# RobertKajnak/AMT-SAGA

Measured on AMD Instinct MI355X. Metric: audio windows/sec (44.1 kHz, 2048-pt STFT) through full detect->subtract loop, higher is better.
Workload: dtype f32 (conv: split-fp16 x2 operands, f32 accumulate; 4x16 layers on the large images in the FFT domain); 1 GPU; C3: 1024 polyphonic piano windows, STFT(2048) + pitch+velocity+timing(start,end) heads + 1 subtraction iteration; windows_per_gpu=1024, n_fft=2048, hop=512, frames=516, iters=1, parallelism=windows sharded x1, event all-gather

## Files before the change

### amt-saga_amd/csrc/amt_conv_f16x3.h

```cpp
#pragma once

typedef _Float16 f16x8 __attribute__((ext_vector_type(8)));
typedef unsigned int u32x2 __attribute__((ext_vector_type(2)));
typedef float f32x4 __attribute__((ext_vector_type(4)));
#define HX_PSTRIDE 80
#define HXS_NIT 2
#define HX_TPITCH 36
#define HX_LSCALE 2048.0f
#define HX_MINNORM 6.103515625e-05f

__host__ __device__ __forceinline__ unsigned short amt_f16_bits(_Float16 h) {
    unsigned short b;
    __builtin_memcpy(&b, &h, 2);
    return b;
}
template <bool FLUSH>
__host__ __device__ __forceinline__ void amt_split_f16(float xs, unsigned short &hb, unsigned short &lb) {
    _Float16 h = (_Float16)xs;
    if (FLUSH && !(__builtin_fabsf(xs) >= HX_MINNORM)) h = (_Float16)0.0f;
    const float r = (xs - (float)h) * HX_LSCALE;
    _Float16 l = (_Float16)r;
    if (FLUSH && !(__builtin_fabsf(r) >= HX_MINNORM)) l = (_Float16)0.0f;
    hb = amt_f16_bits(h);
    lb = amt_f16_bits(l);
// ... 203 lines not shown
            asm volatile("s_waitcnt vmcnt(0)" ::: "memory");
#pragma unroll
            for (int i = 0; i < WPT; ++i) reinterpret_cast<u32x4 *>(wbuf)[tid + i * NT] = wp[i];
            if (NGT > 1) issue(1);
        }
        __syncthreads();
        if (tsp && tid == 0 && ch == 0) tsp[1] = wall_clock64();
        union U { uint4 u; f16x8 v; };
#pragma unroll 1
        for (int g = 0; g < NG; ++g) {
            const int gg = ch * NG + g;
            const uint4 *wb = wbuf + (gg & 1) * GV4 + lane;
            U a[2];
            U b[2][2];
            auto loadA = [&](int tp, int ms) {
                const int tap = g * GT + 2 * tp;
                const int dy = tap / KW, dx = tap - dy * KW;
                const char *ap;
                if constexpr (MASKED) {
                    const int rr = (int)(lrc[ms] & 255u) + dy - PAD_T;
                    const int cc = (int)((lrc[ms] >> 8) & 255u) + dx + tsel - PAD_L;
                    const bool inb = (unsigned)rr < (unsigned)p.H && (unsigned)cc < (unsigned)p.W;
                    ap = in_lds + (inb ? abase[ms] + ((dy - PAD_T) * RP + (dx + tsel - PAD_L)) * HX_PSTRIDE : zero_off);
                } else {
                    ap = in_lds + abase[ms] + (dy * RP + dx) * HX_PSTRIDE;
                }
                a[0].u = *reinterpret_cast<const uint4 *>(ap);
                a[1].u = *reinterpret_cast<const uint4 *>(ap + 32);
            };
            auto mfma6 = [&](int ms) {
#pragma unroll
                for (int ns = 0; ns < 2; ++ns) {
                    lo[ms][ns] = __builtin_amdgcn_mfma_f32_16x16x32_f16(a[1].v, b[ns][0].v, lo[ms][ns], 0, 0, 0);
                    hi[ms][ns] = __builtin_amdgcn_mfma_f32_16x16x32_f16(a[0].v, b[ns][0].v, hi[ms][ns], 0, 0, 0);
                    lo[ms][ns] = __builtin_amdgcn_mfma_f32_16x16x32_f16(a[0].v, b[ns][1].v, lo[ms][ns], 0, 0, 0);
                }
            };
            if constexpr (!MASKED) if (g == NG - 1 && ch + 1 < NCHUNK) stage_issue(ch + 1);
#pragma unroll
            for (int tp = 0; tp < GT / 2; ++tp) {
#pragma unroll
                for (int ns = 0; ns < 2; ++ns)
#pragma unroll
                    for (int pl = 0; pl < 2; ++pl) b[ns][pl].u = wb[((tp * 2 + pl) * 2 + ns) * 64];
#pragma unroll
                for (int ms = 0; ms < MS; ++ms) {
                    loadA(tp, ms);
                    mfma6(ms);
                }
            }
            __builtin_amdgcn_sched_barrier(0);
            if (gg + 1 < NGT) {
                asm volatile("s_waitcnt vmcnt(0)" ::: "memory");
                u32x4 *dst = reinterpret_cast<u32x4 *>(wbuf + ((gg + 1) & 1) * GV4);
#pragma unroll
                for (int i = 0; i < WPT; ++i) dst[tid + i * NT] = wp[i];
                if (gg + 2 < NGT) issue(gg + 2);
            }
            if (g + 1 < NG) __syncthreads();
        }
    }
    if (tsp && tid == 0) tsp[2] = wall_clock64();
    if (tid < PCAP) {
        const int wl = min(max(pos_win[tid] - win0, 0), HX_MAXWIN - 1);
        const int sa = (int)(__float_as_uint(win_is[wl]) >> 23) - 127;
        const int sw = TRAIN ? *hs.sw_dev : hs.sw;
        pos_os[tid] = __uint_as_float((unsigned)(127 - (sa + sw)) << 23);
    }
    __syncthreads();
    float *tb = reinterpret_cast<float *>(in_lds) + wid * (16 * MS * HX_TPITCH);
    const int c4 = (lane & 7) * 4;
    const float4 s2v = *reinterpret_cast<const float4 *>(bnp + 64 + c4), t2v = *reinterpret_cast<const float4 *>(bnp + 96 + c4);
    float osc[MS][4];
#pragma unroll
    for (int ms = 0; ms < MS; ++ms)
#pragma unroll
        for (int e = 0; e < 4; ++e) osc[ms][e] = pos_os[wid * (16 * MS) + ms * 16 + 4 * (lane >> 4) + e];
#pragma unroll
    for (int ns = 0; ns < 2; ++ns) {
        const float s1 = bnp[ns * 16 + (lane & 15)], t1 = bnp[32 + ns * 16 + (lane & 15)];
#pragma unroll
        for (int ms = 0; ms < MS; ++ms)
#pragma unroll
            for (int e = 0; e < 4; ++e) {
                const int row = ms * 16 + 4 * (lane >> 4) + e;
                const float z = (hi[ms][ns][e] + lo[ms][ns][e] * (1.0f / HX_LSCALE)) * osc[ms][e];
                tb[row * HX_TPITCH + ns * 16 + (lane & 15)] = TRAIN ? z + t1 : sigmoidf_(z * s1 + t1);
            }
    }
    constexpr int NR = 2 * MS;
    int spq[NR], gwq[NR];
    float4 scv[NR];
#pragma unroll
    for (int i = 0; i < NR; ++i) {
        const int q = wid * (16 * MS) + (lane >> 3) + 8 * i;
        spq[i] = pos_sp[q];
        gwq[i] = pos_win[q];
    }
    const bool has_sc = p.sc || p.sc1;
    if (p.sc) {
#pragma unroll
        for (int i = 0; i < NR; ++i) {
            const float *scp = p.sc + (size_t)gwq[i] * p.sc_win_stride + (size_t)max(spq[i], 0) * p.cout_total + cout_off + c4;
            scv[i] = spq[i] >= 0 ? *reinterpret_cast<const float4 *>(scp) : make_float4(0.f, 0.f, 0.f, 0.f);
        }
    } else if (p.sc1) {
        const float4 w4 = *reinterpret_cast<const float4 *>(p.sc1_w + cout_off + c4);
        const float4 s4 = *reinterpret_cast<const float4 *>(p.sc1_s + cout_off + c4);
        const float4 t4 = *reinterpret_cast<const float4 *>(p.sc1_t + cout_off + c4);
#pragma unroll
        for (int i = 0; i < NR; ++i) {
            const float x = spq[i] >= 0 ? p.sc1[(size_t)gwq[i] * p.sc1_win_stride + spq[i]] : 0.f;
            scv[i] = make_float4(fmaf(x, w4.x, 0.f) * s4.x + t4.x, fmaf(x, w4.y, 0.f) * s4.y + t4.y,
                                 fmaf(x, w4.z, 0.f) * s4.z + t4.z, fmaf(x, w4.w, 0.f) * s4.w + t4.w);
        }
    }
    float rmax[NR];
#pragma unroll
    for (int i = 0; i < NR; ++i) {
        float4 v = *reinterpret_cast<const float4 *>(tb + ((lane >> 3) + 8 * i) * HX_TPITCH + c4);
        rmax[i] = 0.f;
        if (spq[i] < 0) continue;
        if (has_sc) {
            v.x = (v.x + scv[i].x) * s2v.x + t2v.x;
            v.y = (v.y + scv[i].y) * s2v.y + t2v.y;
            v.z = (v.z + scv[i].z) * s2v.z + t2v.z;
            v.w = (v.w + scv[i].w) * s2v.w + t2v.w;
        }
        rmax[i] = fmaxf(fmaxf(fabsf(v.x), fabsf(v.y)), fmaxf(fabsf(v.z), fabsf(v.w)));
        *reinterpret_cast<float4 *>(p.out + (size_t)gwq[i] * p.out_win_stride + (size_t)spq[i] * p.cout_total + cout_off + c4) = v;
    }
    if (hs.amax_out) {
        if (p.NWIN == 1) {
            float m = 0.f;
#pragma unroll
            for (int i = 0; i < NR; ++i) m = fmaxf(m, rmax[i]);
            m = wave_max(m);
            if (lane == 0) atomicMax(win_max, __float_as_int(m));
        } else {
#pragma unroll
            for (int i = 0; i < NR; ++i) {
                float m = rmax[i];
                m = fmaxf(m, __shfl_xor(m, 1, 64));
                m = fmaxf(m, __shfl_xor(m, 2, 64));
                m = fmaxf(m, __shfl_xor(m, 4, 64));
                if ((lane & 7) == 0 && spq[i] >= 0) atomicMax(win_max + (gwq[i] - win0), __float_as_int(m));
            }
        }
        __syncthreads();
        if (tid < p.NWIN && win0 + tid < p.B) atomicMax(reinterpret_cast<int *>(hs.amax_out) + win0 + tid, win_max[tid]);
    }
    if (tsp && tid == 0) tsp[3] = wall_clock64();
}
```

### amt-saga_amd/csrc/amt_rdcnn.hip

```cpp
#include "amt_common.h"
#include "amt_fftconv.h"
#include "amt_convh.h"
#include "amt_rdcnn_topology.h"
#include <vector>
#include <algorithm>
#include <cmath>
#include <cstdlib>

#include "amt_conv_f32.h"
#include "amt_conv_bf16x6.h"
#include "amt_conv_f16x3.h"
#include "amt_rdcnn_small.h"

#define RD_BN_EPS 1e-3f

struct ConvPlan {
    int TH = 0, TW = 0, NWIN = 1;
    size_t lds = 0;
    int nslice = 1, cw = 0;
    bool masked = false;
    double eff = 0;
    void *w = nullptr;
};
struct ConvOp {
    int cin, cout, H, W, kh, kw;
    float *s1 = nullptr, *t1 = nullptr, *s2 = nullptr, *t2 = nullptr;
    bool residual = false;
    int sc_proj = -1;
    int pool_after = 0;
    ConvPlan f32;
    int MT = 2;
    ConvPlan bf16;
    ConvPlan f16;
    int sw = 0;
    std::vector<float> k_host;
    FcLayer fc;
};
struct ProjOp {
    int cin, cout, H, W, ph, pw, HO, WO;
    float *w = nullptr, *s = nullptr, *t = nullptr;
};
struct Tower {
    int in_h, in_w, ph, pw;
    std::vector<ConvOp> convs;
    std::vector<ProjOp> projs;
    size_t max_act = 0;
    int out_h, out_w, out_c;
};
struct ProfPending { hipEvent_t e0, e1; int tower, layer, windows; };
struct ProfAcc { double ms = 0, windows = 0; long launches = 0; };
struct amt_rdcnn {
    mutable bool prof_on = false;
    mutable std::vector<ProfPending> prof_pending;
    mutable std::vector<hipEvent_t> prof_free;
    mutable std::vector<std::vector<ProfAcc>> prof_acc;
    amt_rdcnn_desc d;
    std::vector<Tower> towers;
    std::vector<void *> allocs;
    float *d1w = nullptr, *d1b = nullptr, *d2w = nullptr, *d2b = nullptr;
    int flat = 0;
    double flops = 0;
    mutable int mode = 0;
};

template <class T>
static int upload(amt_rdcnn *n, const void *h, size_t bytes, T **out) {
    void *d = nullptr;
    if (hipMalloc(&d, bytes) != hipSuccess) return AMT_E_NOMEM;
    n->allocs.push_back(d);
    if (hipMemcpy(d, h, bytes, hipMemcpyHostToDevice) != hipSuccess) return AMT_E_HIP;
    *out = static_cast<T *>(d);
    return AMT_OK;
}
static int upload_folded_bn(amt_rdcnn *n, const float *bn, int c, const float *bias, float **s_out, float **t_out) {
    const float *g = bn, *b = bn + c, *m = bn + 2 * c, *v = bn + 3 * c;
    std::vector<float> s(c), t(c);
    for (int i = 0; i < c; ++i) {
        const float sc = g[i] / sqrtf(v[i] + RD_BN_EPS);
        s[i] = sc;
        t[i] = b[i] + ((bias ? bias[i] : 0.f) - m[i]) * sc;
    }
    const int rc = upload(n, s.data(), c * sizeof(float), s_out);
    return rc != AMT_OK ? rc : upload(n, t.data(), c * sizeof(float), t_out);
}

template <class F>
static void for_each_tile(int H, int W, int pcap, int max_win, F consider) {
    if (H * W <= pcap)
        for (int nw = std::min(pcap / (H * W), max_win); nw >= 1; --nw) consider(H, W, nw);
    for (int TH = 1; TH <= H && TH <= pcap; ++TH) {
        int TW = pcap / TH;
        if (TW > W) TW = W;
        if (TW >= 1) consider(TH, TW, 1);
        const int nct = (W + TW - 1) / TW;
        const int TW2 = (W + nct - 1) / nct;
        if (TW2 >= 1 && TW2 <= TW) consider(TH, TW2, 1);
    }
}

static void choose_tile(ConvOp &c) {
    ConvPlan &p = c.f32;
    double best = -1;
    for (int MT = 2; MT >= 1; --MT) {
        const int pcap = 128 * MT;
        for_each_tile(c.H, c.W, pcap, pcap, [&](int TH, int TW, int NWIN) {
            const size_t posin = (size_t)NWIN * (TH + c.kh - 1) * (TW + c.kw - 1);
            const size_t lds = posin * RD_CSTRIDE * 4 + 2 * (size_t)RD_CC * p.cw * 4 + (size_t)pcap * 8;
            if (lds > 150 * 1024) return;
            const double tiles = (double)((c.H + TH - 1) / TH) * ((c.W + TW - 1) / TW) / NWIN;
            double eff = (double)c.H * c.W / (tiles * pcap);
            if (lds > 78 * 1024) eff *= 0.93;
            if (eff > best + 1e-9) { best = eff; p.TH = TH; p.TW = TW; p.NWIN = NWIN; c.MT = MT; p.lds = lds; p.eff = eff; }
        });
    }
}

template <class F>
static void choose_tile_split(const ConvOp &c, ConvPlan &p, int max_win, F lds_of) {
    double best = -1;
    const int pcap = 256;
    p.masked = false; p.TH = 0;
    if (c.H * c.W <= 64) {
        const int nw = std::min(pcap / (c.H * c.W), max_win);
        const size_t lds = lds_of((size_t)nw * c.H * c.W + 1);
        if (lds <= 79 * 1024) {
            p.masked = true; p.TH = c.H; p.TW = c.W; p.NWIN = nw; p.lds = lds;
            p.eff = (double)nw * c.H * c.W / pcap;
            return;
        }
    }
    for_each_tile(c.H, c.W, pcap, max_win, [&](int TH, int TW, int NWIN) {
        const size_t lds = lds_of((size_t)NWIN * (TH + c.kh - 1) * bx_row_pitch(TW, TW + c.kw - 1));
        if (lds > 79 * 1024) return;
        const double tiles = (double)((c.H + TH - 1) / TH) * ((c.W + TW - 1) / TW) / NWIN;
        const double eff = (double)c.H * c.W / (tiles * pcap);
        if (eff > best + 1e-9) { best = eff; p.TH = TH; p.TW = TW; p.NWIN = NWIN; p.lds = lds; p.eff = eff; }
    });
}
static void choose_tile16(ConvOp &c) {
    const int NT = c.bf16.cw / 32, ntaps = c.kh * c.kw;
    const int tps = (NT == 1 && ntaps % 2 == 0) ? 2 : 1;
    const size_t slab = (size_t)tps * 3 * NT * 64 * 16;
    choose_tile_split(c, c.bf16, 256, [&](size_t npos) { return npos * BX_PSTRIDE + 3 * slab + (size_t)256 * 8; });
}

static unsigned apply_plan(ConvParams &p, const ConvPlan &pl) {
    p.TH = pl.TH; p.TW = pl.TW; p.NWIN = pl.NWIN;
    p.tiles_h = (p.H + p.TH - 1) / p.TH; p.tiles_w = (p.W + p.TW - 1) / p.TW;
    const int groups = (p.B + p.NWIN - 1) / p.NWIN;
    return (unsigned)((size_t)groups * p.tiles_h * p.tiles_w);
}

template <int KH, int KW, int CIN, int COUT, bool MASKED>
static int launch_conv16_t(const ConvOp &c, ConvParams p, hipStream_t st) {
    auto kern = conv_bf16x6_kernel<KH, KW, CIN, COUT, MASKED>;
    static bool attr_set = false;
    if (!attr_set) {
        AMT_HIP_CHECK(hipFuncSetAttribute(reinterpret_cast<const void *>(kern),
                                          hipFuncAttributeMaxDynamicSharedMemorySize, (int)(80 * 1024)));
        attr_set = true;
    }
    const unsigned grid = apply_plan(p, c.bf16);
    kern<<<dim3(grid, c.bf16.nslice), 512, c.bf16.lds, st>>>(p, static_cast<const uint4 *>(c.bf16.w));
    AMT_LAUNCH_CHECK();
    return AMT_OK;
}
template <int KH, int KW>
static int launch_conv16_k(const ConvOp &c, const ConvParams &p, hipStream_t st) {
#define BX_CASE(CI, CO)                                                              \
    if (c.cin == CI && c.bf16.cw == CO)                                              \
        return c.bf16.masked ? launch_conv16_t<KH, KW, CI, CO, true>(c, p, st)          \
                          : launch_conv16_t<KH, KW, CI, CO, false>(c, p, st);
    BX_CASE(32, 32) BX_CASE(32, 64) BX_CASE(64, 64) BX_CASE(128, 64)
#undef BX_CASE
    return AMT_E_UNSUPPORTED;
}
static bool conv_channels_supported(int cin, int cout) {
    return (cin == 32 && cout == 32) || (cin == 32 && cout == 64) || (cin == 64 && cout == 64) ||
           (cin == 64 && cout == 128) || (cin == 128 && cout == 128);
}
static int launch_conv16(const ConvOp &c, const ConvParams &p, hipStream_t st) {
    if (c.kh == 4 && c.kw == 16) return launch_conv16_k<4, 16>(c, p, st);
    if (c.kh == 4 && c.kw == 2) return launch_conv16_k<4, 2>(c, p, st);
    if (c.kh == 2 && c.kw == 2) return launch_conv16_k<2, 2>(c, p, st);
    return AMT_E_UNSUPPORTED;
}


#define HX_SLAB_BYTES 4096
#define HX_XCHG_BYTES (8 * 32 * HX_TPITCH * 4)
static void choose_tile_h(ConvOp &c) {
    const int NTh = c.f16.cw / 32;
    const int nsteps = c.kh * c.kw / (NTh == 1 ? 2 : 1);
    const size_t wbytes = 2 * (size_t)std::min(4, nsteps) * HX_SLAB_BYTES;
    choose_tile_split(c, c.f16, HX_MAXWIN, [&](size_t npos) {
        return std::max(npos * HX_PSTRIDE, (size_t)HX_XCHG_BYTES) + wbytes + (size_t)256 * 12 + (size_t)HX_MAXWIN * 8 + 512;
    });
}

template <int KH, int KW, int CIN, bool MASKED>
static int launch_convs_t(const ConvOp &c, ConvParams p, const float *amax_in, float *amax_out, hipStream_t st) {
    auto kern = conv_f16x3s_kernel<KH, KW, CIN, MASKED>;
    static bool attr_set = false;
    if (!attr_set) {
        AMT_HIP_CHECK(hipFuncSetAttribute(reinterpret_cast<const void *>(kern),
                                          hipFuncAttributeMaxDynamicSharedMemorySize, (int)(80 * 1024)));
        attr_set = true;
    }
    const unsigned grid = apply_plan(p, c.f16);
    HxScale hs{amax_in, amax_out, c.sw, nullptr};
    static const bool want_ts = getenv("AMT_CONV_TS") != nullptr;
    static unsigned long long *ts_dev = nullptr;
    static size_t ts_cap = 0;
    const size_t nwg = (size_t)grid * c.f16.nslice;
    if (want_ts) {
        if (nwg > ts_cap) {
            if (ts_dev) (void)hipFree(ts_dev);
            AMT_HIP_CHECK(hipMalloc(&ts_dev, nwg * 4 * sizeof(unsigned long long)));
            ts_cap = nwg;
        }
        hs.ts = ts_dev;
    }
    kern<<<dim3(grid, c.f16.nslice), 512, c.f16.lds, st>>>(p, static_cast<const uint4 *>(c.f16.w), hs);
    AMT_LAUNCH_CHECK();
    if (want_ts) {
        AMT_HIP_CHECK(hipStreamSynchronize(st));
        std::vector<unsigned long long> h(nwg * 4);
        AMT_HIP_CHECK(hipMemcpy(h.data(), ts_dev, h.size() * sizeof(unsigned long long), hipMemcpyDeviceToHost));
        double a = 0, b = 0, e = 0;
        unsigned long long t0 = ~0ull, t1 = 0;
        for (size_t i = 0; i < nwg; ++i) {
            a += (double)(h[4 * i + 1] - h[4 * i]); b += (double)(h[4 * i + 2] - h[4 * i + 1]);
            e += (double)(h[4 * i + 3] - h[4 * i + 2]);
            t0 = std::min(t0, h[4 * i]); t1 = std::max(t1, h[4 * i + 3]);
        }
        fprintf(stderr, "conv_ts k%dx%d cin%d %dx%d masked%d wgs %zu: start->first MFMA %.2f us, MFMA loop %.2f us, epilogue %.2f us; "
                        "kernel %.1f us = %.2f workgroup lives per slot of 512\n",
                KH, KW, CIN, p.H, p.W, (int)MASKED, nwg, a / nwg / 100.0, b / nwg / 100.0, e / nwg / 100.0,
                (double)(t1 - t0) / 100.0, (double)(t1 - t0) * 512.0 / ((a + b + e)));
    }
    return AMT_OK;
}
template <int KH, int KW>
static int launch_convh_k(const ConvOp &c, const ConvParams &p, const float *amax_in, float *amax_out, hipStream_t st) {
    if (!c.f16.w || c.f16.cw != 32) return AMT_E_UNSUPPORTED;
#define HXS_CASE(CI)                                                                       \
    if (c.cin == CI)                                                                       \
        return c.f16.masked ? launch_convs_t<KH, KW, CI, true>(c, p, amax_in, amax_out, st)               \
                            : launch_convs_t<KH, KW, CI, false>(c, p, amax_in, amax_out, st);
    HXS_CASE(32) HXS_CASE(64) HXS_CASE(128)
#undef HXS_CASE
    return AMT_E_UNSUPPORTED;
}
static int launch_convh(const ConvOp &c, const ConvParams &p, const float *amax_in, float *amax_out, hipStream_t st) {
    if (c.kh == 4 && c.kw == 16) return launch_convh_k<4, 16>(c, p, amax_in, amax_out, st);
    if (c.kh == 4 && c.kw == 2) return launch_convh_k<4, 2>(c, p, amax_in, amax_out, st);
    if (c.kh == 2 && c.kw == 2) return launch_convh_k<2, 2>(c, p, amax_in, amax_out, st);
    return AMT_E_UNSUPPORTED;
}

template <int KH, int KW, int CIN, int COUT, int MT>
static int launch_conv_t(const ConvOp &c, ConvParams p, hipStream_t st) {
    auto kern = conv_mfma_kernel<KH, KW, CIN, COUT, MT>;
    static size_t attr_set = 0;
    if (c.f32.lds > attr_set) {
        AMT_HIP_CHECK(hipFuncSetAttribute(reinterpret_cast<const void *>(kern),
                                          hipFuncAttributeMaxDynamicSharedMemorySize, (int)(152 * 1024)));
        attr_set = 152 * 1024;
    }
    const unsigned grid = apply_plan(p, c.f32);
    kern<<<dim3(grid, c.f32.nslice), 256, c.f32.lds, st>>>(p);
    AMT_LAUNCH_CHECK();
    return AMT_OK;
}

template <int KH, int KW>
static int launch_conv_k(const ConvOp &c, const ConvParams &p, hipStream_t st) {
#define RD_CASE(CI, CO)                                                         \
    if (c.cin == CI && c.f32.cw == CO)                                          \
        return c.MT == 2 ? launch_conv_t<KH, KW, CI, CO, 2>(c, p, st)           \
                         : launch_conv_t<KH, KW, CI, CO, 1>(c, p, st);
    RD_CASE(32, 32) RD_CASE(32, 64) RD_CASE(64, 64) RD_CASE(64, 128) RD_CASE(128, 128)
    RD_CASE(64, 32) RD_CASE(128, 32)
#undef RD_CASE
    return AMT_E_UNSUPPORTED;
}

static int launch_conv(const ConvOp &c, const ConvParams &p, hipStream_t st) {
    if (c.kh == 4 && c.kw == 16) return launch_conv_k<4, 16>(c, p, st);
    if (c.kh == 4 && c.kw == 2) return launch_conv_k<4, 2>(c, p, st);
    if (c.kh == 2 && c.kw == 2) return launch_conv_k<2, 2>(c, p, st);
    return AMT_E_UNSUPPORTED;
}

static void choose_tile1(int H, int W, int *TH_, int *TW_) {
    long best = -1;
    for (int TH = 1; TH <= H && TH <= C1M_PCAP; ++TH) {
        int TWmax = std::min(W, C1M_PCAP / TH);
        for (int TW = std::max(1, TWmax - 40); TW <= TWmax; ++TW) {
            const long tiles = (long)((H + TH - 1) / TH) * ((W + TW - 1) / TW);
            const long cost = tiles * ((TH * TW + 31) / 32);
            if (best < 0 || cost < best) { best = cost; *TH_ = TH; *TW_ = TW; }
        }
    }
}

static bool conv_supported(int kh, int kw) {
    return (kh == 4 && kw == 16) || (kh == 4 && kw == 2) || (kh == 2 && kw == 2);
}

static int launch_conv1_mfma(const ConvOp &c, const Conv1Params &cp, hipStream_t st) {
    int TH1 = 1, TW1 = 1;
    choose_tile1(cp.H, cp.W, &TH1, &TW1);
    const int th = (cp.H + TH1 - 1) / TH1, twn = (cp.W + TW1 - 1) / TW1;
    const size_t lds = (size_t)2 * C1M_PCAP * 4 + (size_t)4 * 32 * HX_TPITCH * 4 +
                       (size_t)(TH1 + c.kh - 1) * (TW1 + c.kw - 1) * 4;
    const unsigned grid = (unsigned)std::min<size_t>((size_t)cp.B * th * twn, 256 * 8);
    if (c.kh == 4 && c.kw == 16) conv1_mfma_kernel<4, 16><<<grid, 256, lds, st>>>(cp, TH1, TW1, th, twn);
    else if (c.kh == 4 && c.kw == 2) conv1_mfma_kernel<4, 2><<<grid, 256, lds, st>>>(cp, TH1, TW1, th, twn);
    else conv1_mfma_kernel<2, 2><<<grid, 256, lds, st>>>(cp, TH1, TW1, th, twn);
    AMT_LAUNCH_CHECK();
    return AMT_OK;
}
static int launch_conv1(const ConvOp &c, const Conv1Params &cp, hipStream_t st) {
    const int groups = 256 / c.cout;
    const size_t lds = ((size_t)c.kh * c.kw * c.cout +
                        (size_t)c.kh * (groups * C1_PPT + c.kw - 1)) * 4;
    const size_t tiles = (size_t)cp.B * cp.H * ((cp.W + groups * C1_PPT - 1) / (groups * C1_PPT));
    conv1_kernel<<<(unsigned)std::min<size_t>(tiles, 8192), 256, lds, st>>>(cp);
    AMT_LAUNCH_CHECK();
    return AMT_OK;
}

enum ConvImpl {
    IMPL_FIRST_MFMA,
    IMPL_FIRST_VALU,
    IMPL_FFT_ROW,
    IMPL_FFT_PACKED,
    IMPL_F16X3,
    IMPL_BF16X6,
    IMPL_F32
};
static ConvImpl conv_impl(const ConvOp &c, int mode) {
    if (c.cin == 1) return (c.cout == 32 && conv_supported(c.kh, c.kw)) ? IMPL_FIRST_MFMA : IMPL_FIRST_VALU;
    if (mode == 3 && c.fc.row) return IMPL_FFT_ROW;
    if (mode == 3 && c.fc.pk) return IMPL_FFT_PACKED;
    if (mode >= 2 && c.f16.w) return IMPL_F16X3;
    if (mode >= 1 && c.bf16.w) return IMPL_BF16X6;
    return IMPL_F32;
}
static bool impl_is_fft(ConvImpl impl) { return impl == IMPL_FFT_ROW || impl == IMPL_FFT_PACKED; }
static bool impl_forms_rank1_shortcut(ConvImpl impl, const ConvOp &c) {
    return impl == IMPL_FFT_ROW || (impl == IMPL_F16X3 && !c.f16.masked);
}
static bool impl_writes_amax(ConvImpl impl) {
    return impl == IMPL_FIRST_MFMA || impl_is_fft(impl) || impl == IMPL_F16X3;
}

static std::vector<float> pack_f32(const float *kern, int ntap, int C, int fo, int nslice) {
    const int nch = C / 32, cw = fo / nslice, NTW = cw / 32;
    std::vector<float> wa((size_t)ntap * C * fo);
    for (int sl = 0; sl < nslice; ++sl)
        for (int ch = 0; ch < nch; ++ch)
            for (int tap = 0; tap < ntap; ++tap)
                for (int cc = 0; cc < 32; ++cc)
                    for (int j = 0; j < 32; ++j)
                        for (int nt = 0; nt < NTW; ++nt)
                            wa[(((((size_t)sl * nch + ch) * ntap + tap) * 32 + cc) * 32 + j) * NTW + nt] =
                                kern[((size_t)tap * C + ch * 32 + cc) * fo + sl * cw + nt * 32 + j];
    return wa;
}
static std::vector<unsigned short> pack_bf16x6(const float *kern, int ntap, int C, int fo, int nslice16) {
    const int NT = fo / 32, cw16 = fo / nslice16, NT16 = cw16 / 32;
    const int tps = (NT16 == 1 && ntap % 2 == 0) ? 2 : 1;
    const int nslab = ntap / tps;
    const int nch16 = C / BX_CC;
    std::vector<unsigned short> w16((size_t)nch16 * ntap * 3 * NT * 2 * 32 * 8);
    for (int sl = 0; sl < nslice16; ++sl)
        for (int ch = 0; ch < nch16; ++ch)
            for (int sb = 0; sb < nslab; ++sb)
                for (int tt = 0; tt < tps; ++tt)
                    for (int nt = 0; nt < NT16; ++nt)
                        for (int h = 0; h < 2; ++h)
                            for (int col = 0; col < 32; ++col)
                                for (int jj = 0; jj < 8; ++jj) {
                                    const int tap = sb * tps + tt;
                                    const int cin_i = ch * BX_CC + 8 * h + jj;
                                    const float wv = kern[((size_t)tap * C + cin_i) * fo + sl * cw16 + nt * 32 + col];
                                    unsigned short hh[3];
                                    amt_split3(wv, hh[0], hh[1], hh[2]);
                                    for (int pl = 0; pl < 3; ++pl) {
                                        const size_t idx =
                                            ((((((((size_t)sl * nch16 + ch) * nslab + sb) * tps + tt) * 3 + pl) * NT16 + nt) * 2 + h) * 32 + col) * 8 + jj;
                                        w16[idx] = hh[pl];
                                    }
                                }
    return w16;
}
static std::vector<unsigned short> pack_f16x3(const float *kern, int ntap, int C, int fo, float wscale) {
    const int NT = fo / 32, nsliceh = fo / 32;
    const int nch16 = C / BX_CC;
    std::vector<unsigned short> ws((size_t)nch16 * ntap * 2 * NT * 2 * 32 * 8);
    const int ntp = ntap / 2;
    for (int sl = 0; sl < nsliceh; ++sl)
        for (int ch = 0; ch < nch16; ++ch)
            for (int tp = 0; tp < ntp; ++tp)
                for (int ns = 0; ns < 2; ++ns)
                    for (int ln = 0; ln < 64; ++ln)
                        for (int jj = 0; jj < 8; ++jj) {
                            const int col = ln & 15, kg = ln >> 4;
                            const int tap = 2 * tp + (kg & 1);
                            const int cin_i = ch * BX_CC + 8 * (kg >> 1) + jj;
                            const float wv = kern[((size_t)tap * C + cin_i) * fo + sl * 32 + ns * 16 + col];
                            unsigned short hh[2];
                            amt_split_f16<true>(wv * wscale, hh[0], hh[1]);
                            for (int pl = 0; pl < 2; ++pl) {
                                const size_t idx =
                                    ((((((size_t)sl * nch16 + ch) * ntp + tp) * 2 + pl) * 2 + ns) * 64 + ln) * 8 + jj;
                                ws[idx] = hh[pl];
                            }
                        }
    return ws;
}

static int build_conv_variants(amt_rdcnn *n, ConvOp &c, const float *kern) {
    const int C = c.cin, fo = c.cout, H = c.H, W = c.W, kh = c.kh, kw = c.kw, ntap = kh * kw;
    if (C % 32 || fo % 32 || !conv_supported(kh, kw) || !conv_channels_supported(C, fo)) return AMT_E_UNSUPPORTED;
    if ((kh == 4 && kw == 16 && C == 32 && fo == 32 && W + 15 <= 576 && H <= 20) ||
        (kh == 4 && kw == 16 && C == 64 && fo == 64 && W == 64 && H == 10))
        c.k_host.assign(kern, kern + (size_t)ntap * C * fo);
    int rc;
    c.f32.nslice = (fo >= 128 && H * W <= 128) ? fo / 32 : 1;
    c.f32.cw = fo / c.f32.nslice;
    const std::vector<float> wa = pack_f32(kern, ntap, C, fo, c.f32.nslice);
    if ((rc = upload(n, wa.data(), wa.size() * sizeof(float), &c.f32.w)) != AMT_OK) return rc;
    choose_tile(c);
    if (c.f32.TH == 0) return AMT_E_UNSUPPORTED;

    c.bf16.nslice = fo > 64 ? fo / 64 : 1;
    c.bf16.cw = fo / c.bf16.nslice;
    choose_tile16(c);
    if (c.bf16.TH > 0 && c.bf16.eff * 2.67 > c.f32.eff * 1.15) {
        const std::vector<unsigned short> w16 = pack_bf16x6(kern, ntap, C, fo, c.bf16.nslice);
        if ((rc = upload(n, w16.data(), w16.size() * 2, &c.bf16.w)) != AMT_OK) return rc;
    }

    c.f16.cw = 32; c.f16.nslice = fo / 32;
    choose_tile_h(c);
    float wmax = 0.f;
    bool finite = true;
    for (size_t q = 0; q < (size_t)ntap * C * fo; ++q) {
        if (!std::isfinite(kern[q])) finite = false;
        wmax = std::max(wmax, fabsf(kern[q]));
    }
    if (c.f16.TH > 0 && finite && wmax > 0.f) {
        int ew = 0;
        (void)frexpf(wmax, &ew);
        c.sw = 4 - ew;
        const std::vector<unsigned short> ws = pack_f16x3(kern, ntap, C, fo, ldexpf(1.0f, c.sw));
        if ((rc = upload(n, ws.data(), ws.size() * 2, &c.f16.w)) != AMT_OK) return rc;
    }
    return AMT_OK;
}

extern "C" {

size_t amt_rdcnn_param_count(const amt_rdcnn_desc *desc) {
    RdTopology tp;
    return desc && amt_rdcnn_topology(*desc, &tp) == AMT_OK ? tp.total : 0;
}

int amt_rdcnn_destroy(amt_rdcnn *net) {
    if (!net) return AMT_OK;
    for (const ProfPending &pp : net->prof_pending) { (void)hipEventDestroy(pp.e0); (void)hipEventDestroy(pp.e1); }
    for (hipEvent_t e : net->prof_free) (void)hipEventDestroy(e);
    for (void *p : net->allocs) (void)hipFree(p);
    for (Tower &t : net->towers)
        for (ConvOp &c : t.convs)
        {
            if (c.fc.row) amt_fftconv_layer_destroy_internal(c.fc.row);
            if (c.fc.pk) amt_fftpk_layer_destroy_internal(c.fc.pk);
        }
    delete net;
    return AMT_OK;
}

int amt_rdcnn_create(amt_rdcnn **out, const amt_rdcnn_desc *desc, const float *wh, size_t n_floats) {
    if (!out || !desc || !wh) return AMT_E_INVALID;
    const amt_rdcnn_desc &d = *desc;
    if (d.n_towers < 1 || d.n_towers > 2 || d.conv_layers < 1 || d.dense_units < 1 ||
        d.output_classes < 1)
        return AMT_E_INVALID;
    RdTopology tp;
    if (amt_rdcnn_topology(d, &tp) != AMT_OK) return AMT_E_UNSUPPORTED;
    if (tp.total != n_floats) return AMT_E_SHAPE;
    if (!tp.shortcut_ok) return AMT_E_UNSUPPORTED;
    amt_rdcnn *n = new amt_rdcnn();
    n->d = d;
    n->flat = tp.flat;
    n->towers.resize(d.n_towers);
    for (int t = 0; t < d.n_towers; ++t) {
        Tower &tw = n->towers[t];
        tw.in_h = d.in_h[t]; tw.in_w = d.in_w[t]; tw.ph = d.pool_h[t]; tw.pw = d.pool_w[t];
        tw.max_act = (size_t)tw.in_h * tw.in_w;
        tw.out_h = tp.out_h[t]; tw.out_w = tp.out_w[t]; tw.out_c = tp.out_c[t];
    }
    int rc = AMT_OK;
#define RD_TRY(x) do { rc = (x); if (rc != AMT_OK) { amt_rdcnn_destroy(n); return rc; } } while (0)
    for (const RdLayer &l : tp.layers) {
        Tower &tw = n->towers[l.tower];
        ConvOp c;
        c.cin = l.cin; c.cout = l.cout; c.H = l.H; c.W = l.W; c.kh = l.kh; c.kw = l.kw;
        const float *kern = wh + l.kernel;
        RD_TRY(upload_folded_bn(n, wh + l.bn, l.cout, wh + l.bias, &c.s1, &c.t1));
        if (l.cin == 1) RD_TRY(upload(n, kern, (size_t)l.kh * l.kw * l.cout * sizeof(float), &c.f32.w));
        else RD_TRY(build_conv_variants(n, c, kern));
        n->flops += 2.0 * l.H * l.W * (double)l.kh * l.kw * l.cin * l.cout;
        tw.max_act = std::max(tw.max_act, (size_t)l.H * l.W * l.cout);
        c.residual = l.residual;
        if (l.residual && l.sc_bn) {
            ProjOp pr;
            pr.cin = l.sC; pr.cout = l.cout; pr.H = l.sH; pr.W = l.sW;
            pr.ph = l.sc_ph; pr.pw = l.sc_pw; pr.HO = l.H; pr.WO = l.W;
            RD_TRY(upload_folded_bn(n, wh + l.sc_bnorm, l.cout, l.sc_proj ? wh + l.sc_bias : nullptr, &pr.s, &pr.t));
            if (l.sc_proj) RD_TRY(upload(n, wh + l.sc_kernel, (size_t)l.sC * l.cout * sizeof(float), &pr.w));
            n->flops += 2.0 * l.H * l.W * (double)l.sC * l.cout;
            c.sc_proj = (int)tw.projs.size();
            tw.projs.push_back(pr);
        }
        if (l.residual) RD_TRY(upload_folded_bn(n, wh + l.res_bn, l.cout, nullptr, &c.s2, &c.t2));
        c.pool_after = l.pool_after ? 1 : 0;
        tw.convs.push_back(c);
    }
    RD_TRY(upload(n, wh + tp.d1_kernel, (size_t)tp.flat * d.dense_units * sizeof(float), &n->d1w));
    RD_TRY(upload(n, wh + tp.d1_bias, (size_t)d.dense_units * sizeof(float), &n->d1b));
    RD_TRY(upload(n, wh + tp.d2_kernel, (size_t)d.dense_units * d.output_classes * sizeof(float), &n->d2w));
    RD_TRY(upload(n, wh + tp.d2_bias, (size_t)d.output_classes * sizeof(float), &n->d2b));
    n->flops += 2.0 * tp.flat * d.dense_units + 2.0 * d.dense_units * d.output_classes;
#undef RD_TRY
    *out = n;
    return AMT_OK;
}

double amt_rdcnn_flops_per_window(const amt_rdcnn *net) { return net ? net->flops : 0.0; }

int amt_rdcnn_set_mode(amt_rdcnn *net, int mode) {
    if (!net || mode < 0 || mode > 3) return AMT_E_INVALID;
    if (mode == 3) {
        for (Tower &t : net->towers)
            for (ConvOp &c : t.convs)
                if (!c.fc && !c.k_host.empty()) {
                    const int rc = c.cin == 64 ? amt_fftpk_layer_create_internal(&c.fc.pk, c.k_host.data())
                                               : amt_fftconv_layer_create_internal(&c.fc.row, c.k_host.data());
                    if (rc != AMT_OK) return rc;
                    c.fc.H = c.H; c.fc.W = c.W;
                }
    }
    net->mode = mode;
    return AMT_OK;
}

int amt_rdcnn_profile(amt_rdcnn *net, int enable) {
    if (!net) return AMT_E_INVALID;
    net->prof_on = enable != 0;
    if (net->prof_acc.empty()) {
        net->prof_acc.resize(net->towers.size());
        for (size_t t = 0; t < net->towers.size(); ++t) net->prof_acc[t].resize(net->towers[t].convs.size());
    }
    return AMT_OK;
}

int amt_rdcnn_profile_read(amt_rdcnn *net, int32_t *desc, double *ms, double *windows,
                           double *flops_per_window, int cap, int *n_rows, int reset) {
    if (!net || !n_rows) return AMT_E_INVALID;
    for (const ProfPending &pp : net->prof_pending) {
        AMT_HIP_CHECK(hipEventSynchronize(pp.e1));
        float e = 0.f;
        AMT_HIP_CHECK(hipEventElapsedTime(&e, pp.e0, pp.e1));
        ProfAcc &a = net->prof_acc[pp.tower][pp.layer];
        a.ms += e; a.windows += pp.windows; a.launches += 1;
        net->prof_free.push_back(pp.e0);
        net->prof_free.push_back(pp.e1);
    }
    net->prof_pending.clear();
    int r = 0;
    for (size_t t = 0; t < net->prof_acc.size(); ++t)
        for (size_t i = 0; i < net->prof_acc[t].size(); ++i) {
            if (r < cap && desc && ms && windows && flops_per_window) {
                const ConvOp &c = net->towers[t].convs[i];
                int32_t *d = desc + (size_t)r * 8;
                d[0] = (int)t; d[1] = (int)i + 1; d[2] = c.kh; d[3] = c.kw; d[4] = c.cin; d[5] = c.cout;
                d[6] = c.H; d[7] = c.W;
                ms[r] = net->prof_acc[t][i].ms;
                windows[r] = net->prof_acc[t][i].windows;
                flops_per_window[r] = 2.0 * c.H * c.W * (double)c.kh * c.kw * c.cin * c.cout;
            }
            ++r;
        }
    *n_rows = r;
    if (reset)
        for (auto &v : net->prof_acc) for (auto &a : v) a = ProfAcc();
// ... 339 lines not shown
```

Before: 13310 windows/s.

## Add window-major f16x3 conv kernel for small masked 4x16 layers

```diff
diff --git a/amt-saga_amd/csrc/amt_conv_f16x3.h b/amt-saga_amd/csrc/amt_conv_f16x3.h
--- a/amt-saga_amd/csrc/amt_conv_f16x3.h
+++ b/amt-saga_amd/csrc/amt_conv_f16x3.h
@@ -379,3 +379,275 @@
     }
     if (tsp && tid == 0) tsp[3] = wall_clock64();
 }
+
+#define HXW_WIN 16
+#define HXW_PPITCH (HXW_WIN * HX_PSTRIDE)
+#define HXW_NWAVE 8
+template <int KW>
+__host__ __device__ constexpr int hxw_group_bytes() { return (KW / 2) * 4096; }
+template <int KW>
+__host__ __device__ constexpr size_t hxw_lds_bytes(int npos) {
+    const size_t tile = (size_t)npos * HXW_PPITCH + HX_PSTRIDE, patch = (size_t)HXW_NWAVE * 16 * HX_TPITCH * 4;
+    return 2 * (size_t)hxw_group_bytes<KW>() + 3 * HXW_WIN * 4 + 512 + (tile > patch ? tile : patch);
+}
+template <int KH, int KW, int CIN, int MS>
+__global__ __launch_bounds__(64 * HXW_NWAVE, 2) void conv_f16x3w_kernel(ConvParams p, const uint4 *__restrict__ w16s, HxScale hs,
+                                                                         int nslice) {
+    constexpr int NT = 64 * HXW_NWAVE;
+    constexpr int NIT = (MS + 1) / 2;
+    constexpr int NCHUNK = CIN / BX_CC;
+    constexpr int PAD_T = (KH - 1) / 2, PAD_L = (KW - 1) / 2;
+    constexpr int NTP = KW / 2;
+    constexpr int GV4 = hxw_group_bytes<KW>() / 16;
+    constexpr int NG = KH, NGT = NCHUNK * NG;
+    constexpr int WPT = GV4 / NT;
+    constexpr int BATCH = MS <= 5 ? MS : 2;
+    constexpr bool PREFETCH = MS <= 5;
+    static_assert(KW % 2 == 0 && NTP <= 8 && GV4 % NT == 0 && MS % BATCH == 0, "whole groups");
+    extern __shared__ __attribute__((aligned(16))) float smem[];
+    uint4 *wbuf = reinterpret_cast<uint4 *>(smem);
+    float *win_is = reinterpret_cast<float *>(wbuf + 2 * GV4);
+    float *win_os = win_is + HXW_WIN;
+    int *win_max = reinterpret_cast<int *>(win_os + HXW_WIN);
+    float *bnp = reinterpret_cast<float *>(win_max + HXW_WIN);
+    char *in_lds = reinterpret_cast<char *>(bnp + 128);
+
+    const int tid = threadIdx.x, lane = tid & 63;
+    const int wid = __builtin_amdgcn_readfirstlane(tid >> 6);
+    unsigned long long *tsp = hs.ts ? hs.ts + (size_t)blockIdx.x * 4 : nullptr;
+    if (tsp && tid == 0) tsp[0] = wall_clock64();
+    const int slice = blockIdx.x % nslice, win0 = (blockIdx.x / nslice) * HXW_WIN;
+    const int cout_off = slice * 32;
+    const uint4 *w16 = w16s + (size_t)slice * ((size_t)NCHUNK * NG * GV4);
+    const int npos = p.H * p.W;
+
+    float my_amax = 0.f;
+    if (tid < HXW_WIN && win0 + tid < p.B) my_amax = hs.amax_in[win0 + tid];
+    float my_bn = 0.f;
+    if (tid < 128) {
+        const float *src = tid < 32 ? p.s1 : tid < 64 ? p.t1 : tid < 96 ? p.s2 : p.t2;
+        my_bn = src ? src[cout_off + (tid & 31)] : ((tid < 32 || (tid >= 64 && tid < 96)) ? 1.f : 0.f);
+    }
+    unsigned rowm[MS], pm[MS], mlane[MS];
+    const int tsel = (lane >> 4) & 1;
+#pragma unroll
+    for (int ms = 0; ms < MS; ++ms) {
+        const int q = wid + HXW_NWAVE * ms;
+        const int r = q / p.W, c = q - r * p.W;
+        unsigned rm = 0, m0 = 0, m1 = 0;
+#pragma unroll
+        for (int dy = 0; dy < KH; ++dy) rm |= (unsigned)((unsigned)(r + dy - PAD_T) < (unsigned)p.H) << dy;
+#pragma unroll
+        for (int tp = 0; tp < NTP; ++tp) {
+            m0 |= (unsigned)((unsigned)(c + 2 * tp - PAD_L) < (unsigned)p.W) << tp;
+            m1 |= (unsigned)((unsigned)(c + 2 * tp + 1 - PAD_L) < (unsigned)p.W) << tp;
+        }
+        rowm[ms] = q < npos ? rm : 0u;
+        pm[ms] = m0 | m1;
+        mlane[ms] = tsel ? m1 : m0;
+    }
+    const int abase = (wid * HXW_WIN + (lane & 15)) * HX_PSTRIDE + (lane >> 5) * 16 + tsel * HXW_PPITCH;
+    const int zero_off = npos * HXW_PPITCH + (lane >> 5) * 16;
+    if (tid < HX_PSTRIDE / 4) reinterpret_cast<unsigned *>(in_lds + npos * HXW_PPITCH)[tid] = 0u;
+    f32x4 hi[MS][2], lo[MS][2];
+#pragma unroll
+    for (int ms = 0; ms < MS; ++ms)
+#pragma unroll
+        for (int ns = 0; ns < 2; ++ns)
+#pragma unroll
+            for (int e = 0; e < 4; ++e) { hi[ms][ns][e] = 0.f; lo[ms][ns][e] = 0.f; }
+
+    u32x4 wp[WPT];
+    auto issue = [&](int gg) {
+        const uint4 *src = w16 + (size_t)gg * GV4 + tid;
+#pragma unroll
+        for (int i = 0; i < WPT; ++i)
+            asm volatile("global_load_dwordx4 %0, %1, off" : "=v"(wp[i]) : "v"(src + i * NT) : "memory");
+    };
+    const int items = npos * HXW_WIN * 2;
+    int sdst[NIT];
+    const float *ssrc[NIT];
+    auto slot_live = [&](int u) { return u * NT + wid * 64 < items; };
+#pragma unroll
+    for (int u = 0; u < NIT; ++u) {
+        const int it = u * NT + tid;
+        sdst[u] = -1; ssrc[u] = nullptr;
+        if (it < items) {
+            const int cg = it & 1, w_ = (it >> 1) & (HXW_WIN - 1), q = it >> 5, gw = win0 + w_;
+            sdst[u] = ((q * HXW_WIN + w_) * HX_PSTRIDE + cg * 16) | (w_ << 24);
+            if (gw < p.B) ssrc[u] = p.in + (size_t)gw * p.in_win_stride + (size_t)q * CIN + cg * 8;
+        }
+    }
+    u32x4 sv[NIT][2];
+    auto stage_issue = [&](int ch) {
+#pragma unroll
+        for (int u = 0; u < NIT; ++u) {
+            if (!slot_live(u)) continue;
+            const float *src = ssrc[u] ? ssrc[u] + ch * BX_CC : p.in;
+            asm volatile("global_load_dwordx4 %0, %1, off" : "=v"(sv[u][0]) : "v"(src) : "memory");
+            asm volatile("global_load_dwordx4 %0, %1, off offset:16" : "=v"(sv[u][1]) : "v"(src) : "memory");
+        }
+    };
+    auto split_store = [&](const float (&v)[8], int dsto, float in_scale) {
+        unsigned short h[2][8];
+#pragma unroll
+        for (int e = 0; e < 8; ++e) amt_split_f16<false>(v[e] * in_scale, h[0][e], h[1][e]);
+        char *dst = in_lds + dsto;
+#pragma unroll
+        for (int pl = 0; pl < 2; ++pl) {
+            uint4 pk;
+            pk.x = h[pl][0] | ((unsigned)h[pl][1] << 16);
+            pk.y = h[pl][2] | ((unsigned)h[pl][3] << 16);
+            pk.z = h[pl][4] | ((unsigned)h[pl][5] << 16);
+            pk.w = h[pl][6] | ((unsigned)h[pl][7] << 16);
+            *reinterpret_cast<uint4 *>(dst + pl * 32) = pk;
+        }
+    };
+    issue(0);
+    if constexpr (PREFETCH) stage_issue(0);
+    if (tid < HXW_WIN) {
+        const int sa = hx_scale_exp(my_amax);
+        win_is[tid] = __uint_as_float((unsigned)(127 + sa) << 23);
+        win_os[tid] = __uint_as_float((unsigned)(127 - (sa + hs.sw)) << 23);
+        win_max[tid] = 0;
+    }
+    if (tid < 128) bnp[tid] = my_bn;
+    for (int ch = 0; ch < NCHUNK; ++ch) {
+        __syncthreads();
+        if constexpr (!PREFETCH) stage_issue(ch);
+        if (ch == 0 || !PREFETCH) asm volatile("s_waitcnt vmcnt(0)" ::: "memory");
+#pragma unroll
+        for (int u = 0; u < NIT; ++u) asm volatile("" : "+v"(sv[u][0]), "+v"(sv[u][1]));
+#pragma unroll
+        for (int u = 0; u < NIT; ++u) {
+            if (sdst[u] < 0 || !slot_live(u)) continue;
+            float v[8];
+#pragma unroll
+            for (int e = 0; e < 8; ++e) v[e] = ssrc[u] ? __uint_as_float(sv[u][e >> 2][e & 3]) : 0.f;
+            split_store(v, sdst[u] & 0xFFFFFF, win_is[sdst[u] >> 24]);
+        }
+        if (ch == 0) {
+#pragma unroll
+            for (int i = 0; i < WPT; ++i) reinterpret_cast<u32x4 *>(wbuf)[tid + i * NT] = wp[i];
+            if (NGT > 1) issue(1);
+        }
+        __syncthreads();
+        if (tsp && tid == 0 && ch == 0) tsp[1] = wall_clock64();
+        union U { uint4 u; f16x8 v; };
+#pragma unroll 1
+        for (int g = 0; g < NG; ++g) {
+            const int gg = ch * NG + g;
+            const uint4 *wb = wbuf + (gg & 1) * GV4 + lane;
+            const int goff = abase + ((g - PAD_T) * p.W - PAD_L) * HXW_PPITCH;
+            unsigned lv[MS], any = 0;
+#pragma unroll
+            for (int ms = 0; ms < MS; ++ms) { lv[ms] = (rowm[ms] >> g) & 1u ? pm[ms] : 0u; any |= lv[ms]; }
+            if (PREFETCH && g == NG - 1 && ch + 1 < NCHUNK) stage_issue(ch + 1);
+            U a[BATCH][2];
+            U b[2][2];
+#pragma unroll
+            for (int tp = 0; tp < NTP; ++tp) {
+                if (!((any >> tp) & 1u)) continue;
+#pragma unroll
+                for (int ns = 0; ns < 2; ++ns)
+#pragma unroll
+                    for (int pl = 0; pl < 2; ++pl) b[ns][pl].u = wb[((tp * 2 + pl) * 2 + ns) * 64];
+#pragma unroll
+                for (int m0 = 0; m0 < MS; m0 += BATCH) {
+#pragma unroll
+                    for (int mb = 0; mb < BATCH; ++mb) {
+                        const int ms = m0 + mb;
+                        if (!((lv[ms] >> tp) & 1u)) continue;
+                        const int off = ((mlane[ms] >> tp) & 1u) ? goff + (ms * HXW_NWAVE + 2 * tp) * HXW_PPITCH : zero_off;
+                        a[mb][0].u = *reinterpret_cast<const uint4 *>(in_lds + off);
+                        a[mb][1].u = *reinterpret_cast<const uint4 *>(in_lds + off + 32);
+                    }
+#pragma unroll
+                    for (int mb = 0; mb < BATCH; ++mb) {
+                        const int ms = m0 + mb;
+                        if (!((lv[ms] >> tp) & 1u)) continue;
+#pragma unroll
+                        for (int ns = 0; ns < 2; ++ns) {
+                            lo[ms][ns] = __builtin_amdgcn_mfma_f32_16x16x32_f16(a[mb][1].v, b[ns][0].v, lo[ms][ns], 0, 0, 0);
+                            hi[ms][ns] = __builtin_amdgcn_mfma_f32_16x16x32_f16(a[mb][0].v, b[ns][0].v, hi[ms][ns], 0, 0, 0);
+                            lo[ms][ns] = __builtin_amdgcn_mfma_f32_16x16x32_f16(a[mb][0].v, b[ns][1].v, lo[ms][ns], 0, 0, 0);
+                        }
+                    }
+                }
+            }
+            __builtin_amdgcn_sched_barrier(0);
+            if (gg + 1 < NGT) {
+                asm volatile("s_waitcnt vmcnt(0)" ::: "memory");
+                u32x4 *dst = reinterpret_cast<u32x4 *>(wbuf + ((gg + 1) & 1) * GV4);
+#pragma unroll
+                for (int i = 0; i < WPT; ++i) dst[tid + i * NT] = wp[i];
+                if (gg + 2 < NGT) issue(gg + 2);
+            }
+            if (g + 1 < NG) __syncthreads();
+        }
+    }
+    if (tsp && tid == 0) tsp[2] = wall_clock64();
+    __syncthreads();
+    float *tb = reinterpret_cast<float *>(in_lds) + wid * (16 * HX_TPITCH);
+    const int c4 = (lane & 7) * 4;
+    const float4 s2v = *reinterpret_cast<const float4 *>(bnp + 64 + c4), t2v = *reinterpret_cast<const float4 *>(bnp + 96 + c4);
+    float osc[4];
+#pragma unroll
+    for (int e = 0; e < 4; ++e) osc[e] = win_os[4 * (lane >> 4) + e];
+    float4 w4 = make_float4(0.f, 0.f, 0.f, 0.f), s4 = w4, t4 = w4;
+    if (p.sc1) {
+        w4 = *reinterpret_cast<const float4 *>(p.sc1_w + cout_off + c4);
+        s4 = *reinterpret_cast<const float4 *>(p.sc1_s + cout_off + c4);
+        t4 = *reinterpret_cast<const float4 *>(p.sc1_t + cout_off + c4);
+    }
+    float rmax[2] = {0.f, 0.f};
+#pragma unroll
+    for (int ms = 0; ms < MS; ++ms) {
+        const int q = wid + HXW_NWAVE * ms;
+        if (q >= npos) continue;
+#pragma unroll
+        for (int ns = 0; ns < 2; ++ns) {
+            const float s1 = bnp[ns * 16 + (lane & 15)], t1 = bnp[32 + ns * 16 + (lane & 15)];
+#pragma unroll
+            for (int e = 0; e < 4; ++e) {
+                const int row = 4 * (lane >> 4) + e;
+                const float z = (hi[ms][ns][e] + lo[ms][ns][e] * (1.0f / HX_LSCALE)) * osc[e];
+                tb[row * HX_TPITCH + ns * 16 + (lane & 15)] = sigmoidf_(z * s1 + t1);
+            }
+        }
+#pragma unroll
+        for (int i = 0; i < 2; ++i) {
+            const int row = (lane >> 3) + 8 * i, gw = win0 + row;
+            float4 v = *reinterpret_cast<const float4 *>(tb + row * HX_TPITCH + c4);
+            if (gw >= p.B) continue;
+            if (p.sc) {
+                const float4 scv = *reinterpret_cast<const float4 *>(p.sc + (size_t)gw * p.sc_win_stride + (size_t)q * p.cout_total + cout_off + c4);
+                v.x = (v.x + scv.x) * s2v.x + t2v.x;
+                v.y = (v.y + scv.y) * s2v.y + t2v.y;
+                v.z = (v.z + scv.z) * s2v.z + t2v.z;
+                v.w = (v.w + scv.w) * s2v.w + t2v.w;
+            } else if (p.sc1) {
+                const float x = p.sc1[(size_t)gw * p.sc1_win_stride + q];
+                v.x = (v.x + (fmaf(x, w4.x, 0.f) * s4.x + t4.x)) * s2v.x + t2v.x;
+                v.y = (v.y + (fmaf(x, w4.y, 0.f) * s4.y + t4.y)) * s2v.y + t2v.y;
+                v.z = (v.z + (fmaf(x, w4.z, 0.f) * s4.z + t4.z)) * s2v.z + t2v.z;
+                v.w = (v.w + (fmaf(x, w4.w, 0.f) * s4.w + t4.w)) * s2v.w + t2v.w;
+            }
+            rmax[i] = fmaxf(rmax[i], fmaxf(fmaxf(fabsf(v.x), fabsf(v.y)), fmaxf(fabsf(v.z), fabsf(v.w))));
+            *reinterpret_cast<float4 *>(p.out + (size_t)gw * p.out_win_stride + (size_t)q * p.cout_total + cout_off + c4) = v;
+        }
+    }
+    if (hs.amax_out) {
+#pragma unroll
+        for (int i = 0; i < 2; ++i) {
+            float m = rmax[i];
+            m = fmaxf(m, __shfl_xor(m, 1, 64));
+            m = fmaxf(m, __shfl_xor(m, 2, 64));
+            m = fmaxf(m, __shfl_xor(m, 4, 64));
+            if ((lane & 7) == 0) atomicMax(win_max + (lane >> 3) + 8 * i, __float_as_int(m));
+        }
+        __syncthreads();
+        if (tid < HXW_WIN && win0 + tid < p.B) atomicMax(reinterpret_cast<int *>(hs.amax_out) + win0 + tid, win_max[tid]);
+    }
+    if (tsp && tid == 0) tsp[3] = wall_clock64();
+}
diff --git a/amt-saga_amd/csrc/amt_rdcnn.hip b/amt-saga_amd/csrc/amt_rdcnn.hip
--- a/amt-saga_amd/csrc/amt_rdcnn.hip
+++ b/amt-saga_amd/csrc/amt_rdcnn.hip
@@ -19,6 +19,8 @@
     size_t lds = 0;
     int nslice = 1, cw = 0;
     bool masked = false;
+    int wm_ms = 0;
+    size_t wm_lds = 0;
     double eff = 0;
     void *w = nullptr;
 };
@@ -198,6 +200,50 @@
     });
 }
 
+static bool conv_ts_wanted() {
+    static const bool want = getenv("AMT_CONV_TS") != nullptr;
+    return want;
+}
+static int conv_ts_buffer(size_t nwg, unsigned long long **out) {
+    static unsigned long long *ts_dev = nullptr;
+    static size_t ts_cap = 0;
+    if (nwg > ts_cap) {
+        if (ts_dev) (void)hipFree(ts_dev);
+        ts_dev = nullptr; ts_cap = 0;
+        AMT_HIP_CHECK(hipMalloc(&ts_dev, nwg * 4 * sizeof(unsigned long long)));
+        ts_cap = nwg;
+    }
+    *out = ts_dev;
+    return AMT_OK;
+}
+static int conv_ts_report(const ConvOp &c, const char *form, const unsigned long long *ts_dev, size_t nwg, int slots, hipStream_t st) {
+    AMT_HIP_CHECK(hipStreamSynchronize(st));
+    std::vector<unsigned long long> h(nwg * 4);
+    AMT_HIP_CHECK(hipMemcpy(h.data(), ts_dev, h.size() * sizeof(unsigned long long), hipMemcpyDeviceToHost));
+    double a = 0, b = 0, e = 0;
+    unsigned long long t0 = ~0ull, t1 = 0;
+    for (size_t i = 0; i < nwg; ++i) {
+        a += (double)(h[4 * i + 1] - h[4 * i]); b += (double)(h[4 * i + 2] - h[4 * i + 1]);
+        e += (double)(h[4 * i + 3] - h[4 * i + 2]);
+        t0 = std::min(t0, h[4 * i]); t1 = std::max(t1, h[4 * i + 3]);
+    }
+    fprintf(stderr, "conv_ts k%dx%d cin%d %dx%d %s wgs %zu: start->first MFMA %.2f us, MFMA loop %.2f us, epilogue %.2f us; "
+                    "kernel %.1f us = %.2f workgroup lives per slot of %d\n",
+            c.kh, c.kw, c.cin, c.H, c.W, form, nwg, a / nwg / 100.0, b / nwg / 100.0, e / nwg / 100.0,
+            (double)(t1 - t0) / 100.0, (double)(t1 - t0) * slots / ((a + b + e)), slots);
+    return AMT_OK;
+}
+static void choose_tile_w(ConvOp &c) {
+    ConvPlan &p = c.f16;
+    p.wm_ms = 0;
+    const char *e = getenv("AMT_CONV_WMAJOR");
+    if (e && e[0] == '0') return;
+    if (!p.masked || c.kh != 4 || c.kw != 16 || !(c.cin == 32 || c.cin == 64 || c.cin == 128)) return;
+    const int npos = c.H * c.W, ms = (npos + HXW_NWAVE - 1) / HXW_NWAVE;
+    p.wm_ms = ms <= 3 ? 3 : ms <= 5 ? 5 : 8;
+    p.wm_lds = hxw_lds_bytes<16>(npos);
+}
+
 template <int KH, int KW, int CIN, bool MASKED>
 static int launch_convs_t(const ConvOp &c, ConvParams p, const float *amax_in, float *amax_out, hipStream_t st) {
     auto kern = conv_f16x3s_kernel<KH, KW, CIN, MASKED>;
@@ -209,37 +255,40 @@
     }
     const unsigned grid = apply_plan(p, c.f16);
     HxScale hs{amax_in, amax_out, c.sw, nullptr};
-    static const bool want_ts = getenv("AMT_CONV_TS") != nullptr;
-    static unsigned long long *ts_dev = nullptr;
-    static size_t ts_cap = 0;
     const size_t nwg = (size_t)grid * c.f16.nslice;
-    if (want_ts) {
-        if (nwg > ts_cap) {
-            if (ts_dev) (void)hipFree(ts_dev);
-            AMT_HIP_CHECK(hipMalloc(&ts_dev, nwg * 4 * sizeof(unsigned long long)));
-            ts_cap = nwg;
-        }
-        hs.ts = ts_dev;
-    }
+    if (conv_ts_wanted()) { const int rc = conv_ts_buffer(nwg, &hs.ts); if (rc != AMT_OK) return rc; }
     kern<<<dim3(grid, c.f16.nslice), 512, c.f16.lds, st>>>(p, static_cast<const uint4 *>(c.f16.w), hs);
     AMT_LAUNCH_CHECK();
-    if (want_ts) {
-        AMT_HIP_CHECK(hipStreamSynchronize(st));
-        std::vector<unsigned long long> h(nwg * 4);
-        AMT_HIP_CHECK(hipMemcpy(h.data(), ts_dev, h.size() * sizeof(unsigned long long), hipMemcpyDeviceToHost));
-        double a = 0, b = 0, e = 0;
-        unsigned long long t0 = ~0ull, t1 = 0;
-        for (size_t i = 0; i < nwg; ++i) {
-            a += (double)(h[4 * i + 1] - h[4 * i]); b += (double)(h[4 * i + 2] - h[4 * i + 1]);
-            e += (double)(h[4 * i + 3] - h[4 * i + 2]);
-            t0 = std::min(t0, h[4 * i]); t1 = std::max(t1, h[4 * i + 3]);
-        }
-        fprintf(stderr, "conv_ts k%dx%d cin%d %dx%d masked%d wgs %zu: start->first MFMA %.2f us, MFMA loop %.2f us, epilogue %.2f us; "
-                        "kernel %.1f us = %.2f workgroup lives per slot of 512\n",
-                KH, KW, CIN, p.H, p.W, (int)MASKED, nwg, a / nwg / 100.0, b / nwg / 100.0, e / nwg / 100.0,
-                (double)(t1 - t0) / 100.0, (double)(t1 - t0) * 512.0 / ((a + b + e)));
-    }
-    return AMT_OK;
+    if (hs.ts) return conv_ts_report(c, MASKED ? "masked1" : "masked0", hs.ts, nwg, 512, st);
+    return AMT_OK;
+}
+template <int KH, int KW, int CIN, int MS>
+static int launch_convw_t(const ConvOp &c, ConvParams p, const float *amax_in, float *amax_out, hipStream_t st) {
+    auto kern = conv_f16x3w_kernel<KH, KW, CIN, MS>;
+    static bool attr_set = false;
+    if (!attr_set) {
+        AMT_HIP_CHECK(hipFuncSetAttribute(reinterpret_cast<const void *>(kern),
+                                          hipFuncAttributeMaxDynamicSharedMemorySize, (int)(160 * 1024)));
+        attr_set = true;
+    }
+    p.TH = p.H; p.TW = p.W; p.NWIN = HXW_WIN; p.tiles_h = p.tiles_w = 1;
+    const size_t nwg = (size_t)((p.B + HXW_WIN - 1) / HXW_WIN) * c.f16.nslice;
+    HxScale hs{amax_in, amax_out, c.sw, nullptr};
+    if (conv_ts_wanted()) { const int rc = conv_ts_buffer(nwg, &hs.ts); if (rc != AMT_OK) return rc; }
+    kern<<<dim3((unsigned)nwg), 64 * HXW_NWAVE, c.f16.wm_lds, st>>>(p, static_cast<const uint4 *>(c.f16.w), hs, c.f16.nslice);
+    AMT_LAUNCH_CHECK();
+    if (hs.ts) return conv_ts_report(c, "wmajor", hs.ts, nwg, 256, st);
+    return AMT_OK;
+}
+static int launch_convw(const ConvOp &c, const ConvParams &p, const float *amax_in, float *amax_out, hipStream_t st) {
+    if (!c.f16.w || c.f16.cw != 32 || c.kh != 4 || c.kw != 16 || c.H * c.W > 8 * c.f16.wm_ms) return AMT_E_UNSUPPORTED;
+#define HXW_CASE(CI, MS)                                                                   \
+    if (c.cin == CI && c.f16.wm_ms == MS) return launch_convw_t<4, 16, CI, MS>(c, p, amax_in, amax_out, st);
+    HXW_CASE(32, 3) HXW_CASE(32, 5) HXW_CASE(32, 8)
+    HXW_CASE(64, 3) HXW_CASE(64, 5) HXW_CASE(64, 8)
+    HXW_CASE(128, 3) HXW_CASE(128, 5) HXW_CASE(128, 8)
+#undef HXW_CASE
+    return AMT_E_UNSUPPORTED;
 }
 template <int KH, int KW>
 static int launch_convh_k(const ConvOp &c, const ConvParams &p, const float *amax_in, float *amax_out, hipStream_t st) {
@@ -253,6 +302,7 @@
     return AMT_E_UNSUPPORTED;
 }
 static int launch_convh(const ConvOp &c, const ConvParams &p, const float *amax_in, float *amax_out, hipStream_t st) {
+    if (c.f16.wm_ms > 0) return launch_convw(c, p, amax_in, amax_out, st);
     if (c.kh == 4 && c.kw == 16) return launch_convh_k<4, 16>(c, p, amax_in, amax_out, st);
     if (c.kh == 4 && c.kw == 2) return launch_convh_k<4, 2>(c, p, amax_in, amax_out, st);
     if (c.kh == 2 && c.kw == 2) return launch_convh_k<2, 2>(c, p, amax_in, amax_out, st);
@@ -351,7 +401,7 @@
 }
 static bool impl_is_fft(ConvImpl impl) { return impl == IMPL_FFT_ROW || impl == IMPL_FFT_PACKED; }
 static bool impl_forms_rank1_shortcut(ConvImpl impl, const ConvOp &c) {
-    return impl == IMPL_FFT_ROW || (impl == IMPL_F16X3 && !c.f16.masked);
+    return impl == IMPL_FFT_ROW || (impl == IMPL_F16X3 && (!c.f16.masked || c.f16.wm_ms > 0));
 }
 static bool impl_writes_amax(ConvImpl impl) {
     return impl == IMPL_FIRST_MFMA || impl_is_fft(impl) || impl == IMPL_F16X3;
@@ -447,6 +497,7 @@
 
     c.f16.cw = 32; c.f16.nslice = fo / 32;
     choose_tile_h(c);
+    choose_tile_w(c);
     float wmax = 0.f;
     bool finite = true;
     for (size_t q = 0; q < (size_t)ntap * C * fo; ++q) {
```

Result: faster. 13580 windows/s (median of 6 runs) (+2.0%).
